# DerrickWang005/CRIS.pytorch

Measured on AMD Instinct MI355X. Metric: train-step samples/sec, CRIS-R50 416x416 bs=64; loss parity vs ref, higher is better.
Workload: dtype bf16; 1 GPU; CRIS-R50 bf16 training step (fwd+BCE+bwd+Adam), 416x416, per-GPU bs=8, 17-token text, synthetic RefCOCO-shape batch resident in HBM (BASELINE.json configs[1]); global_batch=8, parallelism=dp1, launch=graph, graph_captured=True, syncbn_exchange=none, grad_exchange=none

## Files before the change

cris/pytorch_amd/csrc/elementwise.hip:

```cpp
#include <cmath>
#include "common.h"
#include "../../../include/cris_hip.h"

__device__ __forceinline__ void ld8f(const float* p, float* f) {
    const float4 a = *reinterpret_cast<const float4*>(p);
    const float4 b = *reinterpret_cast<const float4*>(p + 4);
    f[0] = a.x; f[1] = a.y; f[2] = a.z; f[3] = a.w; f[4] = b.x; f[5] = b.y; f[6] = b.z; f[7] = b.w;
}
__device__ __forceinline__ void ld8bf(const bf16_t* p, float* f) { unpack8(*reinterpret_cast<const uint4*>(p), f); }
__device__ __forceinline__ void st8bf(bf16_t* p, const float* f) { *reinterpret_cast<uint4*>(p) = pack8(f); }

#define GRID_STRIDE(idx, total) \
    for (long idx = (long)blockIdx.x * blockDim.x + threadIdx.x; idx < (total); idx += (long)gridDim.x * blockDim.x)

__global__ void stem_im2col_kernel(const float* __restrict__ img, int Bn, int H, int W, int OH, int OW, bf16_t* __restrict__ out) {
    const long total = (long)Bn * OH * OW * 4;
    const bool small = total < (1L << 24);
    GRID_STRIDE(idx, total) {
        const cris_idx4 q = cris_split4(idx, 4, OW, OH, small);
        const int kc = q.cv, ow = q.x, oh = q.y, b = q.b;
        const long m = idx >> 2;
        float v[8];
#pragma unroll
        for (int j = 0; j < 8; ++j) {
// ... 41 lines not shown
#pragma unroll
        for (int j = 0; j < 8; ++j) o[j] *= 0.25f;
        st8bf(y + (size_t)mo * ldy + ycoff + cv * 8, o);
    }
}

extern "C" int cris_avgpool2_fwd(const cris_bf16* x, int ldx, int xcoff, int Bn, int H, int W, int C, cris_bf16* y,
                                 int ldy, int ycoff, void* stream) {
    CRIS_CHECK_ARG(x && y && !(H & 1) && !(W & 1) && !(C & 7) && !(ldx & 7) && !(ldy & 7) && !(xcoff & 7) && !(ycoff & 7), "bad args");
    const long total = (long)Bn * (H / 2) * (W / 2) * (C / 8);
    hipLaunchKernelGGL(avgpool2_fwd_kernel, dim3(cris_grid_1d(total, 256)), dim3(256), 0, (hipStream_t)stream, x, ldx, xcoff,
                       Bn, H, W, C, y, ldy, ycoff);
    CRIS_LAUNCH_CHECK();
    return 0;
}

__global__ void avgpool2_bwd_kernel(const bf16_t* __restrict__ dy, int lddy, int dycoff, int Bn, int H, int W, int C,
                                    bf16_t* __restrict__ dx, int lddx, int dxcoff, int accum) {
    const int CV = C >> 3, OH = H >> 1, OW = W >> 1;
    const long total = (long)Bn * H * W * CV;
    const bool small = total < (1L << 24);
    GRID_STRIDE(idx, total) {
        const cris_idx4 q = cris_split4(idx, CV, W, H, small);
        const int cv = q.cv, w = q.x, h = q.y, b = q.b;
        const long m = ((long)b * H + h) * W + w;
        float g[8];
        ld8bf(dy + (((size_t)b * OH + (h >> 1)) * OW + (w >> 1)) * lddy + dycoff + cv * 8, g);
        bf16_t* d = dx + (size_t)m * lddx + dxcoff + cv * 8;
        float o[8];
        if (accum) ld8bf(d, o);
#pragma unroll
        for (int j = 0; j < 8; ++j) o[j] = (accum ? o[j] : 0.f) + 0.25f * g[j];
        st8bf(d, o);
    }
}

extern "C" int cris_avgpool2_bwd(const cris_bf16* dy, int lddy, int dycoff, int Bn, int H, int W, int C, cris_bf16* dx,
                                 int lddx, int dxcoff, int accum, void* stream) {
    CRIS_CHECK_ARG(dy && dx && !(H & 1) && !(W & 1) && !(C & 7) && !(lddx & 7) && !(lddy & 7) && !(dxcoff & 7) && !(dycoff & 7), "bad args");
    const long total = (long)Bn * H * W * (C / 8);
    hipLaunchKernelGGL(avgpool2_bwd_kernel, dim3(cris_grid_1d(total, 256)), dim3(256), 0, (hipStream_t)stream, dy, lddy, dycoff,
                       Bn, H, W, C, dx, lddx, dxcoff, accum);
    CRIS_LAUNCH_CHECK();
    return 0;
}

__device__ __forceinline__ void up2_src(int dst, int n_in, int& i0, int& i1, float& l1) {
    float s = (dst + 0.5f) * 0.5f - 0.5f;
    s = fmaxf(s, 0.f);
    i0 = (int)s;
    i1 = i0 < n_in - 1 ? i0 + 1 : i0;
    l1 = s - (float)i0;
}

__global__ void upsample2_fwd_kernel(const bf16_t* __restrict__ x, int ldx, int xcoff, int Bn, int H, int W, int C,
                                     bf16_t* __restrict__ y, int ldy, int ycoff) {
    const int CV = C >> 3, OH = H * 2, OW = W * 2;
    const long total = (long)Bn * OH * OW * CV;
    const bool small = total < (1L << 24);
    GRID_STRIDE(idx, total) {
        const cris_idx4 q = cris_split4(idx, CV, OW, OH, small);
        const int cv = q.cv, ow = q.x, oh = q.y, b = q.b;
        const long mo = ((long)b * OH + oh) * OW + ow;
        int y0, y1, x0, x1;
        float ly, lx;
        up2_src(oh, H, y0, y1, ly);
        up2_src(ow, W, x0, x1, lx);
        const bf16_t* base = x + (size_t)b * H * W * ldx + xcoff + cv * 8;
        float a[8], bb[8], c[8], d[8], o[8];
        ld8bf(base + ((size_t)y0 * W + x0) * ldx, a);
        ld8bf(base + ((size_t)y0 * W + x1) * ldx, bb);
        ld8bf(base + ((size_t)y1 * W + x0) * ldx, c);
        ld8bf(base + ((size_t)y1 * W + x1) * ldx, d);
        const float w00 = (1.f - ly) * (1.f - lx), w01 = (1.f - ly) * lx, w10 = ly * (1.f - lx), w11 = ly * lx;
#pragma unroll
        for (int j = 0; j < 8; ++j) o[j] = w00 * a[j] + w01 * bb[j] + w10 * c[j] + w11 * d[j];
        st8bf(y + (size_t)mo * ldy + ycoff + cv * 8, o);
    }
}

extern "C" int cris_upsample2_fwd(const cris_bf16* x, int ldx, int xcoff, int Bn, int H, int W, int C, cris_bf16* y,
                                  int ldy, int ycoff, void* stream) {
    CRIS_CHECK_ARG(x && y && !(C & 7) && !(ldx & 7) && !(ldy & 7) && !(xcoff & 7) && !(ycoff & 7), "bad args");
    const long total = (long)Bn * H * W * 4 * (C / 8);
    hipLaunchKernelGGL(upsample2_fwd_kernel, dim3(cris_grid_1d(total, 256)), dim3(256), 0, (hipStream_t)stream, x, ldx, xcoff,
                       Bn, H, W, C, y, ldy, ycoff);
    CRIS_LAUNCH_CHECK();
    return 0;
}

__global__ void upsample2_bwd_kernel(const bf16_t* __restrict__ dy, int lddy, int dycoff, int Bn, int H, int W, int C,
                                     bf16_t* __restrict__ dx, int lddx, int dxcoff, int accum) {
    const int CV = C >> 3, OH = H * 2, OW = W * 2;
    const long total = (long)Bn * H * W * CV;
    const bool small = total < (1L << 24);
    GRID_STRIDE(idx, total) {
        const cris_idx4 q = cris_split4(idx, CV, W, H, small);
        const int cv = q.cv, ix = q.x, iy = q.y, b = q.b;
        const long m = ((long)b * H + iy) * W + ix;
        float acc[8] = {0, 0, 0, 0, 0, 0, 0, 0};
        const bf16_t* base = dy + (size_t)b * OH * OW * lddy + dycoff + cv * 8;
        for (int oy = max(0, 2 * iy - 2); oy <= min(OH - 1, 2 * iy + 2); ++oy) {
            int y0, y1; float ly;
            up2_src(oy, H, y0, y1, ly);
            float wy = 0.f;
            if (y0 == iy) wy += 1.f - ly;
            if (y1 == iy) wy += ly;
            if (wy == 0.f) continue;
            for (int ox = max(0, 2 * ix - 2); ox <= min(OW - 1, 2 * ix + 2); ++ox) {
                int x0, x1; float lx;
                up2_src(ox, W, x0, x1, lx);
                float wx = 0.f;
                if (x0 == ix) wx += 1.f - lx;
                if (x1 == ix) wx += lx;
                if (wx == 0.f) continue;
                float g[8];
                ld8bf(base + ((size_t)oy * OW + ox) * lddy, g);
                const float w = wy * wx;
#pragma unroll
                for (int j = 0; j < 8; ++j) acc[j] += w * g[j];
            }
        }
        bf16_t* d = dx + (size_t)m * lddx + dxcoff + cv * 8;
        if (accum) {
            float o[8];
            ld8bf(d, o);
#pragma unroll
            for (int j = 0; j < 8; ++j) acc[j] += o[j];
        }
        st8bf(d, acc);
    }
}

extern "C" int cris_upsample2_bwd(const cris_bf16* dy, int lddy, int dycoff, int Bn, int H, int W, int C, cris_bf16* dx,
                                  int lddx, int dxcoff, int accum, void* stream) {
    CRIS_CHECK_ARG(dy && dx && !(C & 7) && !(lddx & 7) && !(lddy & 7) && !(dxcoff & 7) && !(dycoff & 7), "bad args");
    const long total = (long)Bn * H * W * (C / 8);
    hipLaunchKernelGGL(upsample2_bwd_kernel, dim3(cris_grid_1d(total, 256)), dim3(256), 0, (hipStream_t)stream, dy, lddy, dycoff,
                       Bn, H, W, C, dx, lddx, dxcoff, accum);
    CRIS_LAUNCH_CHECK();
    return 0;
}

__device__ __forceinline__ float linspace_m1_1(int i, int n) {
    if (n == 1) return -1.f;
    const float step = 2.f / (float)(n - 1);
    return i < n / 2 ? -1.f + step * (float)i : 1.f - step * (float)(n - 1 - i);
}

__global__ void fill_coords_kernel(bf16_t* x, int ldx, int coff, int nfill, int Bn, int H, int W) {
    const long total = (long)Bn * H * W;
    GRID_STRIDE(m, total) {
        const int w = (int)(m % W);
        const int h = (int)((m / W) % H);
        bf16_t* d = x + (size_t)m * ldx + coff;
        d[0] = f2bf(linspace_m1_1(w, W));
        d[1] = f2bf(linspace_m1_1(h, H));
        for (int j = 2; j < nfill; ++j) d[j] = 0;
    }
}

extern "C" int cris_fill_coords(cris_bf16* x, int ldx, int coff, int nfill, int Bn, int H, int W, void* stream) {
    CRIS_CHECK_ARG(x && nfill >= 2, "bad args");
    hipLaunchKernelGGL(fill_coords_kernel, dim3(cris_grid_1d((long)Bn * H * W, 256)), dim3(256), 0, (hipStream_t)stream, x, ldx,
                       coff, nfill, Bn, H, W);
    CRIS_LAUNCH_CHECK();
    return 0;
}

__global__ void gather_samples_kernel(const bf16_t* __restrict__ x, int ldx, int xcoff, const int32_t* __restrict__ index,
                                      int R, int CV, bf16_t* __restrict__ y, int ldy, int ycoff, int total) {
    for (int idx = blockIdx.x * blockDim.x + threadIdx.x; idx < total; idx += gridDim.x * blockDim.x) {
        const int cv = idx % CV;
        const int row = idx / CV;
        const int k = row / R;
// ... 315 lines not shown
    const long total = (long)T * C;
    GRID_STRIDE(idx, total) {
        const int c = (int)(idx % C);
        const int t = (int)(idx / C);
        float s = 0.f;
#pragma unroll 7
        for (int j = 0; j < GG; ++j) s += R[t * GG + j] * pos[(size_t)(1 + j) * C + c];
        posr[idx] = s;
    }
}
extern "C" int cris_posresize_fwd(const float* R, const float* pos, int T, int G, int C, float* posr, void* stream) {
    CRIS_CHECK_ARG(R && pos && posr, "bad args");
    hipLaunchKernelGGL(posresize_fwd_kernel, dim3(cris_grid_1d((long)T * C, 256)), dim3(256), 0, (hipStream_t)stream, R, pos, T,
                       G * G, C, posr);
    CRIS_LAUNCH_CHECK();
    return 0;
}
__global__ void posresize_bwd_kernel(const float* R, const float* dposr, int T, int GG, int C, float* dpos) {
    const long total = (long)GG * C;
    GRID_STRIDE(idx, total) {
        const int c = (int)(idx % C);
        const int j = (int)(idx / C);
        float s = 0.f;
#pragma unroll 13
        for (int t = 0; t < T; ++t) s += R[t * GG + j] * dposr[(size_t)t * C + c];
        dpos[(size_t)(1 + j) * C + c] += s;
    }
}
extern "C" int cris_posresize_bwd(const float* R, const float* dposr, int T, int G, int C, float* dpos, void* stream) {
    CRIS_CHECK_ARG(R && dposr && dpos, "bad args");
    hipLaunchKernelGGL(posresize_bwd_kernel, dim3(cris_grid_1d((long)G * G * C, 256)), dim3(256), 0, (hipStream_t)stream, R,
                       dposr, T, G * G, C, dpos);
    CRIS_LAUNCH_CHECK();
    return 0;
}
__global__ void batch_rowsum_kernel(const bf16_t* dx, int ldx, int Bn, int T, int C, float* out) {
    const long total = (long)T * C;
    GRID_STRIDE(idx, total) {
        const int c = (int)(idx % C);
        const int t = (int)(idx / C);
        float s = 0.f;
        for (int b = 0; b < Bn; ++b) s += bf2f(dx[((size_t)b * T + t) * ldx + c]);
        out[idx] = s;
    }
}
extern "C" int cris_batch_rowsum(const cris_bf16* dx, int ldx, int Bn, int T, int C, float* out, void* stream) {
    CRIS_CHECK_ARG(dx && out, "bad args");
    hipLaunchKernelGGL(batch_rowsum_kernel, dim3(cris_grid_1d((long)T * C, 256)), dim3(256), 0, (hipStream_t)stream, dx, ldx, Bn,
                       T, C, out);
    CRIS_LAUNCH_CHECK();
    return 0;
}

__global__ __launch_bounds__(256) void dynconv_fwd_kernel(const bf16_t* __restrict__ x, int H, int W, int C, const float* __restrict__ wb,
                                                          int ldwb, float* __restrict__ pred, int pix_per_block) {
    const int b = blockIdx.y;
    const int LP = C >> 3;
    const int cl = threadIdx.x % LP, sub = threadIdx.x / LP, nsub = 256 / LP;
    float w[9][8];
    const float* wp = wb + (size_t)b * ldwb;
#pragma unroll
    for (int t = 0; t < 9; ++t)
#pragma unroll
        for (int j = 0; j < 8; ++j) w[t][j] = wp[(cl * 8 + j) * 9 + t];
    const float bias = wp[C * 9];
    const int HW = H * W;
    const int p0 = blockIdx.x * pix_per_block;
    const int p1 = min(HW, p0 + pix_per_block);
    for (int pb = p0; pb < p1; pb += nsub) {
        const int pix = pb + sub;
        float acc = 0.f;
        if (pix < p1) {
            const int oh = pix / W, ow = pix - oh * W;
#pragma unroll
            for (int kh = 0; kh < 3; ++kh)
#pragma unroll
                for (int kw = 0; kw < 3; ++kw) {
                    const int ih = oh + kh - 1, iw = ow + kw - 1;
                    const float ok = ((unsigned)ih < (unsigned)H && (unsigned)iw < (unsigned)W) ? 1.f : 0.f;
                    const int ihc = min(max(ih, 0), H - 1), iwc = min(max(iw, 0), W - 1);
                    float v[8];
                    ld8bf(x + (((size_t)b * H + ihc) * W + iwc) * C + cl * 8, v);
#pragma unroll
                    for (int j = 0; j < 8; ++j) acc += ok * v[j] * w[kh * 3 + kw][j];
                }
        }
        for (int o = LP >> 1; o > 0; o >>= 1) acc += __shfl_xor(acc, o, 64);
        if (cl == 0 && pix < p1) pred[(size_t)b * HW + pix] = acc + bias;
    }
}

extern "C" int cris_dynconv_fwd(const cris_bf16* x, int Bn, int H, int W, int C, const float* wb, int ldwb, float* pred,
                                void* stream) {
    const int LP = C / 8;
    CRIS_CHECK_ARG(x && wb && pred && !(C & 7) && LP >= 1 && LP <= 64 && (LP & (LP - 1)) == 0, "C/8 must be a power of two <= 64");
    constexpr int ppb = 128;
    dim3 grid(cris_cdiv(H * W, ppb), Bn);
    hipLaunchKernelGGL(dynconv_fwd_kernel, grid, dim3(256), 0, (hipStream_t)stream, x, H, W, C, wb, ldwb, pred, ppb);
    CRIS_LAUNCH_CHECK();
    return 0;
}

__global__ __launch_bounds__(256) void dynconv_bwd_kernel(const bf16_t* __restrict__ x, const float* __restrict__ dpred, int H, int W, int C,
                                                          const float* __restrict__ wb, int ldwb, bf16_t* __restrict__ dx,
                                                          float* __restrict__ dwb_part, int pix_per_block) {
    extern __shared__ float sdw[];
    const int b = blockIdx.y;
    const int LP = C >> 3;
    const int cl = threadIdx.x % LP, sub = threadIdx.x / LP, nsub = 256 / LP;
    for (int i = threadIdx.x; i < C * 9 + 1; i += 256) sdw[i] = 0.f;
    __syncthreads();
    float w[9][8], dw[9][8];
    const float* wp = wb + (size_t)b * ldwb;
#pragma unroll
    for (int t = 0; t < 9; ++t)
#pragma unroll
        for (int j = 0; j < 8; ++j) {
            w[t][j] = wp[(cl * 8 + j) * 9 + t];
            dw[t][j] = 0.f;
        }
    float dbias = 0.f;
    const int HW = H * W;
    const float* dp = dpred + (size_t)b * HW;
    const int p0 = blockIdx.x * pix_per_block;
    const int p1 = min(HW, p0 + pix_per_block);
    for (int pix = p0 + sub; pix < p1; pix += nsub) {
        const int ph = pix / W, pw = pix - ph * W;
        float gx[8] = {0, 0, 0, 0, 0, 0, 0, 0};
        const float g0 = dp[pix];
        if (cl == 0) dbias += g0;
        float xq[8];
        ld8bf(x + ((size_t)b * HW + pix) * C + cl * 8, xq);
#pragma unroll
        for (int kh = 0; kh < 3; ++kh)
#pragma unroll
            for (int kw = 0; kw < 3; ++kw) {
                const int oh = ph - kh + 1, ow = pw - kw + 1;
                const float okg = ((unsigned)oh < (unsigned)H && (unsigned)ow < (unsigned)W) ? 1.f : 0.f;
                const float g = okg * dp[min(max(oh, 0), H - 1) * W + min(max(ow, 0), W - 1)];
#pragma unroll
                for (int j = 0; j < 8; ++j) {
                    gx[j] += g * w[kh * 3 + kw][j];
                    dw[kh * 3 + kw][j] += g * xq[j];
                }
            }
        st8bf(dx + ((size_t)b * HW + pix) * C + cl * 8, gx);
    }
    for (int o = LP; o < 64; o <<= 1) {
#pragma unroll
        for (int t = 0; t < 9; ++t)
#pragma unroll
            for (int j = 0; j < 8; ++j) dw[t][j] += __shfl_xor(dw[t][j], o, 64);
        dbias += __shfl_xor(dbias, o, 64);
    }
    const int lane = threadIdx.x & 63;
    for (int w = 0; w < 4; ++w) {
        if ((int)(threadIdx.x >> 6) == w && lane < LP) {
#pragma unroll
            for (int t = 0; t < 9; ++t)
#pragma unroll
                for (int j = 0; j < 8; ++j) sdw[(cl * 8 + j) * 9 + t] += dw[t][j];
            if (cl == 0) sdw[C * 9] += dbias;
        }
        __syncthreads();
    }
    float* part = dwb_part + ((size_t)blockIdx.x * gridDim.y + b) * ldwb;
    for (int i = threadIdx.x; i < ldwb; i += 256) part[i] = i < C * 9 + 1 ? sdw[i] : 0.f;
}

#define DYNCONV_BWD_PPB 128
static int dynconv_bwd_blocks(int HW) { return cris_cdiv(HW, DYNCONV_BWD_PPB); }
extern "C" long cris_dynconv_bwd_ws_floats(int Bn, int H, int W, int ldwb) { return (long)dynconv_bwd_blocks(H * W) * Bn * ldwb; }
void cris_launch_sum_partials(const float* part, int nparts, int ncol, float* out, hipStream_t stream);

extern "C" int cris_dynconv_bwd(const cris_bf16* x, const float* dpred, int Bn, int H, int W, int C, const float* wb, int ldwb,
                                cris_bf16* dx, float* dwb, float* ws, void* stream) {
    const int LP = C / 8;
    CRIS_CHECK_ARG(x && dpred && wb && dx && dwb && ws && !(C & 7) && LP >= 1 && LP <= 64 && (LP & (LP - 1)) == 0 && ldwb >= C * 9 + 1,
                   "bad args");
    const int ppb = DYNCONV_BWD_PPB;
    dim3 grid(dynconv_bwd_blocks(H * W), Bn);
    hipLaunchKernelGGL(dynconv_bwd_kernel, grid, dim3(256), (size_t)(C * 9 + 1) * sizeof(float), (hipStream_t)stream, x, dpred, H, W,
                       C, wb, ldwb, dx, ws, ppb);
    CRIS_LAUNCH_CHECK();
    cris_launch_sum_partials(ws, grid.x, Bn * ldwb, dwb, (hipStream_t)stream);
    CRIS_LAUNCH_CHECK();
    return 0;
}

__global__ void mask_resize_kernel(const float* mask, int Bn, int IH, int IW, int OH, int OW, float* out) {
    const float sh = (float)IH / (float)OH, sw = (float)IW / (float)OW;
    const long total = (long)Bn * OH * OW;
    GRID_STRIDE(idx, total) {
        const int ow = (int)(idx % OW);
        const int oh = (int)((idx / OW) % OH);
        const int b = (int)(idx / ((long)OW * OH));
        const int ih = min((int)floorf(oh * sh), IH - 1);
        const int iw = min((int)floorf(ow * sw), IW - 1);
        out[idx] = mask[((size_t)b * IH + ih) * IW + iw];
    }
}
extern "C" int cris_mask_resize_nearest(const float* mask, int Bn, int IH, int IW, int OH, int OW, float* out, void* stream) {
    CRIS_CHECK_ARG(mask && out, "bad args");
    hipLaunchKernelGGL(mask_resize_kernel, dim3(cris_grid_1d((long)Bn * OH * OW, 256)), dim3(256), 0, (hipStream_t)stream, mask, Bn,
                       IH, IW, OH, OW, out);
    CRIS_LAUNCH_CHECK();
    return 0;
}

#define BCE_BLOCKS 128
__global__ __launch_bounds__(256) void bce_fwd_kernel(const float* x, const float* t, long n, float* part) {
    __shared__ float sw[4];
    float s = 0.f;
    const long n4 = n >> 2;
    for (long i = (long)blockIdx.x * 256 + threadIdx.x; i < n4; i += (long)BCE_BLOCKS * 256) {
        const float4 v = *reinterpret_cast<const float4*>(x + i * 4);
        const float4 y = *reinterpret_cast<const float4*>(t + i * 4);
        s += fmaxf(v.x, 0.f) - v.x * y.x + log1pf(__expf(-fabsf(v.x)));
        s += fmaxf(v.y, 0.f) - v.y * y.y + log1pf(__expf(-fabsf(v.y)));
        s += fmaxf(v.z, 0.f) - v.z * y.z + log1pf(__expf(-fabsf(v.z)));
// ... 537 lines not shown
```

cris/pytorch_amd/csrc/norm.hip:

```cpp
#include "common.h"
#include "../../../include/cris_hip.h"
#include "p2p_ll.h"
#include <string.h>

#define BN_WIDE_MIN 128
#define BN_MERGE_MIN 512
#define BN_MERGE_SLICES 64

template <int PL>
__device__ __forceinline__ float bn_lane_sum(float (*sh)[17], float v, int pl, int cl) {
    __syncthreads();
    sh[pl][cl] = v;
    __syncthreads();
    if (PL == 64) {
        float g = 0.f;
        if (pl < 8) {
#pragma unroll
            for (int j = 0; j < 8; ++j) g += sh[pl * 8 + j][cl];
        }
        __syncthreads();
        if (pl < 8) sh[pl][cl] = g;
        __syncthreads();
    }
    float t = sh[0][cl];
// ... 1049 lines not shown
            p.mean[row] = mean;
            p.rstd[row] = rstd;
        }
#pragma unroll
        for (int i = 0; i < LN_MAXV; ++i) {
            const int c0 = (lane + 64 * i) * 8;
            if (c0 >= p.C) continue;
            float ga[8], be[8], o[8];
            load8f(p.gamma + c0, ga);
            load8f(p.beta + c0, be);
#pragma unroll
            for (int j = 0; j < 8; ++j) o[j] = (v[i][j] - mean) * rstd * ga[j] + be[j];
            const size_t oo = (size_t)row * p.C + c0;
            if (p.y) cris_st16(p.y + oo, pack8(o));
            if (p.ypos) {
                float pe[8], t[8];
                load8f(p.pos + (size_t)(row % p.pos_rows) * p.C + c0, pe);
#pragma unroll
                for (int j = 0; j < 8; ++j) t[j] = o[j] + pe[j];
                cris_st16(p.ypos + oo, pack8(t));
            }
            if (p.out_f32) {
                float r[8];
                if (p.resid) load8f(p.resid + oo, r);
                else {
#pragma unroll
                    for (int j = 0; j < 8; ++j) r[j] = 0.f;
                }
#pragma unroll
                for (int j = 0; j < 8; ++j) {
                    float t = o[j];
                    if (p.out_thresh) t = cris_keep(out_key, (uint32_t)row * (uint32_t)p.C + (uint32_t)(c0 + j), p.out_thresh) ? t * out_scale : 0.f;
                    r[j] += t;
                }
                *reinterpret_cast<float4*>(p.out_f32 + oo) = make_float4(r[0], r[1], r[2], r[3]);
                *reinterpret_cast<float4*>(p.out_f32 + oo + 4) = make_float4(r[4], r[5], r[6], r[7]);
            }
        }
    }
}

extern "C" int cris_ln_fwd(const cris_ln_fwd_params* pp, void* stream) {
    const cris_ln_fwd_params& p = *pp;
    CRIS_CHECK_ARG(p.x && p.gamma && p.beta && p.mean && p.rstd && p.rows > 0, "null operand");
    CRIS_CHECK_ARG((p.C & 7) == 0 && p.C <= 64 * 8 * LN_MAXV && (p.ldx & 7) == 0, "C must be a multiple of 8, <= 2048");
    CRIS_CHECK_ARG(!p.ypos || (p.pos && p.pos_rows > 0), "ypos needs pos");
    CRIS_CHECK_ARG((long)p.rows * p.C < (1L << 32), "dropout index overflow");
    const int grid = cris_grid_1d(p.rows, 4, 2048);
    hipLaunchKernelGGL(ln_fwd_kernel, dim3(grid), dim3(256), 0, (hipStream_t)stream, p);
    CRIS_LAUNCH_CHECK();
    return 0;
}

template <int V>
__global__ __launch_bounds__(256) void ln_bwd_kernel(const cris_ln_bwd_params p) {
    __shared__ float sg[2][64 * 8 * V];
    const int lane = threadIdx.x & 63;
    const int wave_g = blockIdx.x * 4 + (threadIdx.x >> 6);
    const int nwaves = gridDim.x * 4;
    for (int i = threadIdx.x; i < 2 * 64 * 8 * V; i += 256) (&sg[0][0])[i] = 0.f;
    __syncthreads();
    const uint32_t sdev = p.seed_dev ? p.seed_dev[0] : 0u;
    const uint32_t in_key = cris_drop_key(p.in_seed + sdev, p.in_stream);
    const uint32_t out_key = cris_drop_key(p.out_seed + sdev, p.out_stream);
    const float in_scale = p.in_thresh ? 1.f / (1.f - p.in_drop_p) : 1.f;
    const float out_scale = p.out_thresh ? 1.f / (1.f - p.out_drop_p) : 1.f;
    const float invC = 1.f / (float)p.C;
    float dga[V][8], dbe[V][8];
#pragma unroll
    for (int i = 0; i < V; ++i)
#pragma unroll
        for (int j = 0; j < 8; ++j) dga[i][j] = dbe[i][j] = 0.f;

    for (int row = wave_g; row < p.rows; row += nwaves) {
        float v[V][8], msk[V][8];
        ln_load_row<true, V>(p.x, p.x_f32, (size_t)row * p.ldx, p.C, lane, p.in_relu, p.in_thresh, in_scale, in_key, (uint32_t)row,
                          v, msk);
        const float mean = p.mean[row], rstd = p.rstd[row];
        float a[V][8];
        float s1 = 0.f, s2 = 0.f;
#pragma unroll
        for (int i = 0; i < V; ++i) {
            const int c0 = (lane + 64 * i) * 8;
            if (c0 < p.C) {
                const size_t oo = (size_t)row * p.C + c0;
                float g[8], t[8], ga[8];
#pragma unroll
                for (int j = 0; j < 8; ++j) g[j] = 0.f;
                if (p.dy) {
                    load8bf(p.dy + oo, t);
#pragma unroll
                    for (int j = 0; j < 8; ++j) g[j] += t[j];
                }
                if (p.dypos) {
                    load8bf(p.dypos + oo, t);
#pragma unroll
                    for (int j = 0; j < 8; ++j) g[j] += t[j];
                }
                if (p.dout_f32) {
                    load8f(p.dout_f32 + oo, t);
#pragma unroll
                    for (int j = 0; j < 8; ++j) {
                        float d = t[j];
                        if (p.out_thresh) d = cris_keep(out_key, (uint32_t)row * (uint32_t)p.C + (uint32_t)(c0 + j), p.out_thresh) ? d * out_scale : 0.f;
                        g[j] += d;
                    }
                }
                load8f(p.gamma + c0, ga);
#pragma unroll
                for (int j = 0; j < 8; ++j) {
                    const float xh = (v[i][j] - mean) * rstd;
                    v[i][j] = xh;
                    dga[i][j] += g[j] * xh;
                    dbe[i][j] += g[j];
                    a[i][j] = g[j] * ga[j];
                    s1 += a[i][j];
                    s2 += a[i][j] * xh;
                }
            } else {
#pragma unroll
                for (int j = 0; j < 8; ++j) a[i][j] = 0.f;
            }
        }
        const float m1 = wave_sum(s1) * invC, m2 = wave_sum(s2) * invC;
#pragma unroll
        for (int i = 0; i < V; ++i) {
            const int c0 = (lane + 64 * i) * 8;
            if (c0 >= p.C) continue;
            float o[8];
#pragma unroll
            for (int j = 0; j < 8; ++j) o[j] = rstd * (a[i][j] - m1 - v[i][j] * m2) * msk[i][j];
            const size_t xo = (size_t)row * p.ldx + c0;
            if (p.dx_f32) {
                float* d = reinterpret_cast<float*>(p.dx) + xo;
                if (p.dx_accum) {
                    float old[8];
                    load8f(d, old);
#pragma unroll
                    for (int j = 0; j < 8; ++j) o[j] += old[j];
                }
                *reinterpret_cast<float4*>(d) = make_float4(o[0], o[1], o[2], o[3]);
                *reinterpret_cast<float4*>(d + 4) = make_float4(o[4], o[5], o[6], o[7]);
            } else {
                cris_st16(reinterpret_cast<bf16_t*>(p.dx) + xo, pack8(o));
            }
        }
    }
    for (int w = 0; w < 4; ++w) {
        if ((int)(threadIdx.x >> 6) == w) {
#pragma unroll
            for (int i = 0; i < V; ++i) {
                const int c0 = (lane + 64 * i) * 8;
                if (c0 < p.C) {
#pragma unroll
                    for (int j = 0; j < 8; ++j) {
                        sg[0][c0 + j] += dga[i][j];
                        sg[1][c0 + j] += dbe[i][j];
                    }
                }
            }
        }
        __syncthreads();
    }
    float* part = p.part + (size_t)blockIdx.x * 2 * p.C;
    for (int c = threadIdx.x; c < p.C; c += 256) {
        part[c] = sg[0][c];
        part[p.C + c] = sg[1][c];
    }
}

constexpr int LN_BWD_BLOCKS = 512;
static int ln_bwd_grid(int rows) { return cris_grid_1d(rows, 4, LN_BWD_BLOCKS); }
extern "C" int cris_ln_bwd_parts(int rows) { return ln_bwd_grid(rows); }

extern "C" int cris_ln_bwd(const cris_ln_bwd_params* pp, void* stream) {
    const cris_ln_bwd_params& p = *pp;
    CRIS_CHECK_ARG(p.x && p.gamma && p.mean && p.rstd && p.dx && p.part && p.rows > 0, "null operand");
    CRIS_CHECK_ARG(p.dy || p.dypos || p.dout_f32, "no incoming gradient");
    CRIS_CHECK_ARG((p.C & 7) == 0 && p.C <= 64 * 8 * LN_MAXV && (p.ldx & 7) == 0, "C must be a multiple of 8, <= 2048");
    CRIS_CHECK_ARG(!p.dx_accum || p.dx_f32, "accumulate only into fp32");
    static const int narrow = cris_env_int("CRIS_LN_BWD_V", 1);
    const dim3 grid(ln_bwd_grid(p.rows));
    if (narrow && p.C <= 512) hipLaunchKernelGGL(ln_bwd_kernel<1>, grid, dim3(256), 0, (hipStream_t)stream, p);
    else if (narrow && p.C <= 1024) hipLaunchKernelGGL(ln_bwd_kernel<2>, grid, dim3(256), 0, (hipStream_t)stream, p);
    else hipLaunchKernelGGL(ln_bwd_kernel<LN_MAXV>, grid, dim3(256), 0, (hipStream_t)stream, p);
    CRIS_LAUNCH_CHECK();
    return 0;
}

__global__ __launch_bounds__(256) void sum_group_kernel(const cris_sum_group g) {
    __shared__ float sh[4][64];
    int ei = 0;
#pragma unroll
    for (int i = 1; i < CRIS_SUM_GROUP_MAX; ++i) ei += g.block_start[i] <= (int)blockIdx.x ? 1 : 0;
    const cris_sum_entry e = g.e[ei];
    const int cl = threadIdx.x & 63, pl = threadIdx.x >> 6;
    const int c = (blockIdx.x - g.block_start[ei]) * 64 + cl;
    float a = 0.f;
    if (c < e.ncol)
        for (int i = pl; i < e.nparts; i += 4) a += e.part[(size_t)i * e.ld + c];
    sh[pl][cl] = a;
    __syncthreads();
    if (pl == 0 && c < e.ncol) e.out[c] = (sh[0][cl] + sh[1][cl]) + (sh[2][cl] + sh[3][cl]);
}

extern "C" int cris_sum_tables(const cris_sum_group* gp, void* stream) {
    CRIS_CHECK_ARG(gp && gp->n > 0 && gp->n <= CRIS_SUM_GROUP_MAX, "1 .. CRIS_SUM_GROUP_MAX tables per launch");
    cris_sum_group g = *gp;
    int start = 0;
    for (int i = 0; i < g.n; ++i) {
        CRIS_CHECK_ARG(g.e[i].part && g.e[i].out && g.e[i].nparts > 0 && g.e[i].ncol > 0 && g.e[i].ld >= g.e[i].ncol, "bad table");
        g.block_start[i] = start;
        start += cris_cdiv(g.e[i].ncol, 64);
    }
    for (int i = g.n; i <= CRIS_SUM_GROUP_MAX; ++i) g.block_start[i] = start;
    hipLaunchKernelGGL(sum_group_kernel, dim3(start), dim3(256), 0, (hipStream_t)stream, g);
    CRIS_LAUNCH_CHECK();
    return 0;
}
```

Baseline: 679.0 samples/s.

## Restructure upsample, dynconv and layernorm-backward kernels for register reuse and batching

Upsample2 forward now has each thread load one 2x2 source neighbourhood and write the up to four output pixels that share it, instead of doing four loads per output. Upsample2 backward replaces its branchy gather loop with a fixed 4x4 unrolled gather using precomputed weights and predication. Dynconv forward computes runs of 4 adjacent pixels from a shared register window and sizes its grid adaptively. Dynconv backward batches 4 pixels' loads ahead of compute and moves shared-memory dW to a vectorised transposed layout. LayerNorm backward keeps per-wave gamma/beta partials in shared memory instead of registers, packs the dropout mask into bits, and adds a full-width specialisation with occupancy hints. The cost is more register pressure and redundant clamped loads at borders.

Result: no change. 683.5 samples/s (median of 6 runs) (+0.7%).

```diff
diff --git a/cris/pytorch_amd/csrc/elementwise.hip b/cris/pytorch_amd/csrc/elementwise.hip
--- a/cris/pytorch_amd/csrc/elementwise.hip
+++ b/cris/pytorch_amd/csrc/elementwise.hip
@@ -117,37 +117,62 @@
     i1 = i0 < n_in - 1 ? i0 + 1 : i0;
     l1 = s - (float)i0;
 }
+__device__ __forceinline__ float up2_tap(int dst, int n_in, int src) {
+    int i0, i1;
+    float l1;
+    up2_src(dst, n_in, i0, i1, l1);
+    float w = 0.f;
+    if (i0 == src) w += 1.f - l1;
+    if (i1 == src) w += l1;
+    return w;
+}
 
 __global__ void upsample2_fwd_kernel(const bf16_t* __restrict__ x, int ldx, int xcoff, int Bn, int H, int W, int C,
                                      bf16_t* __restrict__ y, int ldy, int ycoff) {
-    const int CV = C >> 3, OH = H * 2, OW = W * 2;
-    const long total = (long)Bn * OH * OW * CV;
+    const int CV = C >> 3, OH = H * 2, OW = W * 2, QH = H + 1, QW = W + 1;
+    const long total = (long)Bn * QH * QW * CV;
     const bool small = total < (1L << 24);
     GRID_STRIDE(idx, total) {
-        const cris_idx4 q = cris_split4(idx, CV, OW, OH, small);
-        const int cv = q.cv, ow = q.x, oh = q.y, b = q.b;
-        const long mo = ((long)b * OH + oh) * OW + ow;
-        int y0, y1, x0, x1;
-        float ly, lx;
-        up2_src(oh, H, y0, y1, ly);
-        up2_src(ow, W, x0, x1, lx);
+        const cris_idx4 q = cris_split4(idx, CV, QW, QH, small);
+        const int cv = q.cv, kx = q.x, ky = q.y, b = q.b;
+        const int r0 = max(ky - 1, 0), r1 = ky == 0 ? min(1, H - 1) : min(ky, H - 1);
+        const int c0 = max(kx - 1, 0), c1 = kx == 0 ? min(1, W - 1) : min(kx, W - 1);
         const bf16_t* base = x + (size_t)b * H * W * ldx + xcoff + cv * 8;
-        float a[8], bb[8], c[8], d[8], o[8];
-        ld8bf(base + ((size_t)y0 * W + x0) * ldx, a);
-        ld8bf(base + ((size_t)y0 * W + x1) * ldx, bb);
-        ld8bf(base + ((size_t)y1 * W + x0) * ldx, c);
-        ld8bf(base + ((size_t)y1 * W + x1) * ldx, d);
-        const float w00 = (1.f - ly) * (1.f - lx), w01 = (1.f - ly) * lx, w10 = ly * (1.f - lx), w11 = ly * lx;
-#pragma unroll
-        for (int j = 0; j < 8; ++j) o[j] = w00 * a[j] + w01 * bb[j] + w10 * c[j] + w11 * d[j];
-        st8bf(y + (size_t)mo * ldy + ycoff + cv * 8, o);
+        float a[8], bb[8], c[8], d[8];
+        ld8bf(base + ((size_t)r0 * W + c0) * ldx, a);
+        ld8bf(base + ((size_t)r0 * W + c1) * ldx, bb);
+        ld8bf(base + ((size_t)r1 * W + c0) * ldx, c);
+        ld8bf(base + ((size_t)r1 * W + c1) * ldx, d);
+#pragma unroll
+        for (int dy = 0; dy < 2; ++dy) {
+            const int oh = 2 * ky - 1 + dy;
+            if (oh < 0 || oh >= OH) continue;
+            int y0, y1;
+            float ly;
+            up2_src(oh, H, y0, y1, ly);
+#pragma unroll
+            for (int dx = 0; dx < 2; ++dx) {
+                const int ow = 2 * kx - 1 + dx;
+                if (ow < 0 || ow >= OW) continue;
+                int x0, x1;
+                float lx;
+                up2_src(ow, W, x0, x1, lx);
+                const float w00 = (1.f - ly) * (1.f - lx), w01 = (1.f - ly) * lx, w10 = ly * (1.f - lx), w11 = ly * lx;
+                float o[8];
+#pragma unroll
+                for (int j = 0; j < 8; ++j) o[j] = w00 * a[j] + w01 * bb[j] + w10 * c[j] + w11 * d[j];
+                const long mo = ((long)b * OH + oh) * OW + ow;
+                st8bf(y + (size_t)mo * ldy + ycoff + cv * 8, o);
+            }
+        }
     }
 }
 
 extern "C" int cris_upsample2_fwd(const cris_bf16* x, int ldx, int xcoff, int Bn, int H, int W, int C, cris_bf16* y,
                                   int ldy, int ycoff, void* stream) {
     CRIS_CHECK_ARG(x && y && !(C & 7) && !(ldx & 7) && !(ldy & 7) && !(xcoff & 7) && !(ycoff & 7), "bad args");
-    const long total = (long)Bn * H * W * 4 * (C / 8);
+    if (Bn <= 0 || H <= 0 || W <= 0 || C <= 0) return 0;
+    const long total = (long)Bn * (H + 1) * (W + 1) * (C / 8);
     hipLaunchKernelGGL(upsample2_fwd_kernel, dim3(cris_grid_1d(total, 256)), dim3(256), 0, (hipStream_t)stream, x, ldx, xcoff,
                        Bn, H, W, C, y, ldy, ycoff);
     CRIS_LAUNCH_CHECK();
@@ -165,27 +190,38 @@
         const long m = ((long)b * H + iy) * W + ix;
         float acc[8] = {0, 0, 0, 0, 0, 0, 0, 0};
         const bf16_t* base = dy + (size_t)b * OH * OW * lddy + dycoff + cv * 8;
-        for (int oy = max(0, 2 * iy - 2); oy <= min(OH - 1, 2 * iy + 2); ++oy) {
-            int y0, y1; float ly;
-            up2_src(oy, H, y0, y1, ly);
-            float wy = 0.f;
-            if (y0 == iy) wy += 1.f - ly;
-            if (y1 == iy) wy += ly;
-            if (wy == 0.f) continue;
-            for (int ox = max(0, 2 * ix - 2); ox <= min(OW - 1, 2 * ix + 2); ++ox) {
-                int x0, x1; float lx;
-                up2_src(ox, W, x0, x1, lx);
-                float wx = 0.f;
-                if (x0 == ix) wx += 1.f - lx;
-                if (x1 == ix) wx += lx;
-                if (wx == 0.f) continue;
+        int oyc[4], oxc[4];
+        float wy[4], wx[4];
+        bool oky[4], okx[4];
+#pragma unroll
+        for (int t = 0; t < 4; ++t) {
+            const int oy = 2 * iy - 1 + t, ox = 2 * ix - 1 + t;
+            oky[t] = oy >= 0 && oy < OH;
+            okx[t] = ox >= 0 && ox < OW;
+            oyc[t] = min(max(oy, 0), OH - 1);
+            oxc[t] = min(max(ox, 0), OW - 1);
+            wy[t] = up2_tap(oyc[t], H, iy);
+            wx[t] = up2_tap(oxc[t], W, ix);
+        }
+        uint4 gv[4][4];
+#pragma unroll
+        for (int ty = 0; ty < 4; ++ty)
+#pragma unroll
+            for (int tx = 0; tx < 4; ++tx) gv[ty][tx] = *reinterpret_cast<const uint4*>(base + ((size_t)oyc[ty] * OW + oxc[tx]) * lddy);
+#pragma unroll
+        for (int ty = 0; ty < 4; ++ty)
+#pragma unroll
+            for (int tx = 0; tx < 4; ++tx) {
                 float g[8];
-                ld8bf(base + ((size_t)oy * OW + ox) * lddy, g);
-                const float w = wy * wx;
-#pragma unroll
-                for (int j = 0; j < 8; ++j) acc[j] += w * g[j];
+                unpack8(gv[ty][tx], g);
+                const float w = wy[ty] * wx[tx];
+                const bool ok = oky[ty] && okx[tx];
+#pragma unroll
+                for (int j = 0; j < 8; ++j) {
+                    const float s = acc[j] + w * g[j];
+                    acc[j] = ok ? s : acc[j];
+                }
             }
-        }
         bf16_t* d = dx + (size_t)m * lddx + dxcoff + cv * 8;
         if (accum) {
             float o[8];
@@ -607,8 +643,10 @@
     return 0;
 }
 
+#define DYNCONV_RUN 4
 __global__ __launch_bounds__(256) void dynconv_fwd_kernel(const bf16_t* __restrict__ x, int H, int W, int C, const float* __restrict__ wb,
-                                                          int ldwb, float* __restrict__ pred, int pix_per_block) {
+                                                          int ldwb, float* __restrict__ pred, int runs_per_block) {
+    constexpr int T = DYNCONV_RUN;
     const int b = blockIdx.y;
     const int LP = C >> 3;
     const int cl = threadIdx.x % LP, sub = threadIdx.x / LP, nsub = 256 / LP;
@@ -620,28 +658,44 @@
         for (int j = 0; j < 8; ++j) w[t][j] = wp[(cl * 8 + j) * 9 + t];
     const float bias = wp[C * 9];
     const int HW = H * W;
-    const int p0 = blockIdx.x * pix_per_block;
-    const int p1 = min(HW, p0 + pix_per_block);
-    for (int pb = p0; pb < p1; pb += nsub) {
-        const int pix = pb + sub;
-        float acc = 0.f;
-        if (pix < p1) {
-            const int oh = pix / W, ow = pix - oh * W;
+    const int WR = (W + T - 1) / T;
+    const int r0 = blockIdx.x * runs_per_block;
+    const int r1 = min(H * WR, r0 + runs_per_block);
+    for (int rb = r0; rb < r1; rb += nsub) {
+        const int run = rb + sub;
+        const bool act = run < r1;
+        const int oh = act ? run / WR : 0, ow0 = act ? (run - oh * WR) * T : 0;
+        float acc[T];
+#pragma unroll
+        for (int t = 0; t < T; ++t) acc[t] = 0.f;
+        if (act) {
+            uint4 xv[3][T + 2];
 #pragma unroll
             for (int kh = 0; kh < 3; ++kh)
 #pragma unroll
-                for (int kw = 0; kw < 3; ++kw) {
-                    const int ih = oh + kh - 1, iw = ow + kw - 1;
-                    const float ok = ((unsigned)ih < (unsigned)H && (unsigned)iw < (unsigned)W) ? 1.f : 0.f;
-                    const int ihc = min(max(ih, 0), H - 1), iwc = min(max(iw, 0), W - 1);
-                    float v[8];
-                    ld8bf(x + (((size_t)b * H + ihc) * W + iwc) * C + cl * 8, v);
-#pragma unroll
-                    for (int j = 0; j < 8; ++j) acc += ok * v[j] * w[kh * 3 + kw][j];
+                for (int c = 0; c < T + 2; ++c) {
+                    const int ihc = min(max(oh + kh - 1, 0), H - 1), iwc = min(max(ow0 + c - 1, 0), W - 1);
+                    xv[kh][c] = *reinterpret_cast<const uint4*>(x + (((size_t)b * H + ihc) * W + iwc) * C + cl * 8);
                 }
-        }
-        for (int o = LP >> 1; o > 0; o >>= 1) acc += __shfl_xor(acc, o, 64);
-        if (cl == 0 && pix < p1) pred[(size_t)b * HW + pix] = acc + bias;
+#pragma unroll
+            for (int t = 0; t < T; ++t)
+#pragma unroll
+                for (int kh = 0; kh < 3; ++kh)
+#pragma unroll
+                    for (int kw = 0; kw < 3; ++kw) {
+                        const int ih = oh + kh - 1, iw = ow0 + t + kw - 1;
+                        const float ok = ((unsigned)ih < (unsigned)H && (unsigned)iw < (unsigned)W) ? 1.f : 0.f;
+                        float v[8];
+                        unpack8(xv[kh][t + kw], v);
+#pragma unroll
+                        for (int j = 0; j < 8; ++j) acc[t] += ok * v[j] * w[kh * 3 + kw][j];
+                    }
+        }
+#pragma unroll
+        for (int t = 0; t < T; ++t) {
+            for (int o = LP >> 1; o > 0; o >>= 1) acc[t] += __shfl_xor(acc[t], o, 64);
+            if (cl == 0 && act && ow0 + t < W) pred[(size_t)b * HW + oh * W + ow0 + t] = acc[t] + bias;
+        }
     }
 }
 
@@ -649,17 +703,22 @@
                                 void* stream) {
     const int LP = C / 8;
     CRIS_CHECK_ARG(x && wb && pred && !(C & 7) && LP >= 1 && LP <= 64 && (LP & (LP - 1)) == 0, "C/8 must be a power of two <= 64");
-    constexpr int ppb = 128;
-    dim3 grid(cris_cdiv(H * W, ppb), Bn);
-    hipLaunchKernelGGL(dynconv_fwd_kernel, grid, dim3(256), 0, (hipStream_t)stream, x, H, W, C, wb, ldwb, pred, ppb);
-    CRIS_LAUNCH_CHECK();
-    return 0;
-}
-
+    CRIS_CHECK_ARG(Bn > 0 && H > 0 && W > 0, "empty operand");
+    const int nsub = 256 / LP, runs = H * cris_cdiv(W, DYNCONV_RUN);
+    int rpb = cris_cdiv((long)runs * Bn, 512);
+    if (rpb < 32) rpb = 32;
+    rpb = cris_cdiv(rpb, nsub) * nsub;
+    dim3 grid(cris_cdiv(runs, rpb), Bn);
+    hipLaunchKernelGGL(dynconv_fwd_kernel, grid, dim3(256), 0, (hipStream_t)stream, x, H, W, C, wb, ldwb, pred, rpb);
+    CRIS_LAUNCH_CHECK();
+    return 0;
+}
+
+#define DYNCONV_BWD_BATCH 4
 __global__ __launch_bounds__(256) void dynconv_bwd_kernel(const bf16_t* __restrict__ x, const float* __restrict__ dpred, int H, int W, int C,
                                                           const float* __restrict__ wb, int ldwb, bf16_t* __restrict__ dx,
                                                           float* __restrict__ dwb_part, int pix_per_block) {
-    extern __shared__ float sdw[];
+    extern __shared__ __attribute__((aligned(16))) float sdw[];
     const int b = blockIdx.y;
     const int LP = C >> 3;
     const int cl = threadIdx.x % LP, sub = threadIdx.x / LP, nsub = 256 / LP;
@@ -679,27 +738,40 @@
     const float* dp = dpred + (size_t)b * HW;
     const int p0 = blockIdx.x * pix_per_block;
     const int p1 = min(HW, p0 + pix_per_block);
-    for (int pix = p0 + sub; pix < p1; pix += nsub) {
-        const int ph = pix / W, pw = pix - ph * W;
-        float gx[8] = {0, 0, 0, 0, 0, 0, 0, 0};
-        const float g0 = dp[pix];
-        if (cl == 0) dbias += g0;
-        float xq[8];
-        ld8bf(x + ((size_t)b * HW + pix) * C + cl * 8, xq);
-#pragma unroll
-        for (int kh = 0; kh < 3; ++kh)
-#pragma unroll
-            for (int kw = 0; kw < 3; ++kw) {
-                const int oh = ph - kh + 1, ow = pw - kw + 1;
-                const float okg = ((unsigned)oh < (unsigned)H && (unsigned)ow < (unsigned)W) ? 1.f : 0.f;
-                const float g = okg * dp[min(max(oh, 0), H - 1) * W + min(max(ow, 0), W - 1)];
+    constexpr int D = DYNCONV_BWD_BATCH;
+    for (int pb = p0 + sub; pb < p1; pb += nsub * D) {
+        uint4 xr[D];
+        float g[D][9];
+#pragma unroll
+        for (int d = 0; d < D; ++d) {
+            const int pix = min(pb + d * nsub, p1 - 1);
+            const int ph = pix / W, pw = pix - ph * W;
+            xr[d] = *reinterpret_cast<const uint4*>(x + ((size_t)b * HW + pix) * C + cl * 8);
+#pragma unroll
+            for (int kh = 0; kh < 3; ++kh)
+#pragma unroll
+                for (int kw = 0; kw < 3; ++kw) {
+                    const int oh = ph - kh + 1, ow = pw - kw + 1;
+                    const float okg = ((unsigned)oh < (unsigned)H && (unsigned)ow < (unsigned)W) ? 1.f : 0.f;
+                    g[d][kh * 3 + kw] = okg * dp[min(max(oh, 0), H - 1) * W + min(max(ow, 0), W - 1)];
+                }
+        }
+#pragma unroll
+        for (int d = 0; d < D; ++d) {
+            const int pix = pb + d * nsub;
+            if (pix >= p1) break;
+            float gx[8] = {0, 0, 0, 0, 0, 0, 0, 0}, xq[8];
+            unpack8(xr[d], xq);
+            if (cl == 0) dbias += g[d][4];
+#pragma unroll
+            for (int t = 0; t < 9; ++t)
 #pragma unroll
                 for (int j = 0; j < 8; ++j) {
-                    gx[j] += g * w[kh * 3 + kw][j];
-                    dw[kh * 3 + kw][j] += g * xq[j];
+                    gx[j] += g[d][t] * w[t][j];
+                    dw[t][j] += g[d][t] * xq[j];
                 }
-            }
-        st8bf(dx + ((size_t)b * HW + pix) * C + cl * 8, gx);
+            st8bf(dx + ((size_t)b * HW + pix) * C + cl * 8, gx);
+        }
     }
     for (int o = LP; o < 64; o <<= 1) {
 #pragma unroll
@@ -712,15 +784,23 @@
     for (int w = 0; w < 4; ++w) {
         if ((int)(threadIdx.x >> 6) == w && lane < LP) {
 #pragma unroll
-            for (int t = 0; t < 9; ++t)
-#pragma unroll
-                for (int j = 0; j < 8; ++j) sdw[(cl * 8 + j) * 9 + t] += dw[t][j];
+            for (int t = 0; t < 9; ++t) {
+                float4* q = reinterpret_cast<float4*>(sdw + t * C + cl * 8);
+                float4 lo = q[0], hi = q[1];
+                lo.x += dw[t][0]; lo.y += dw[t][1]; lo.z += dw[t][2]; lo.w += dw[t][3];
+                hi.x += dw[t][4]; hi.y += dw[t][5]; hi.z += dw[t][6]; hi.w += dw[t][7];
+                q[0] = lo;
+                q[1] = hi;
+            }
             if (cl == 0) sdw[C * 9] += dbias;
         }
         __syncthreads();
     }
     float* part = dwb_part + ((size_t)blockIdx.x * gridDim.y + b) * ldwb;
-    for (int i = threadIdx.x; i < ldwb; i += 256) part[i] = i < C * 9 + 1 ? sdw[i] : 0.f;
+    for (int i = threadIdx.x; i < ldwb; i += 256) {
+        const int c = i / 9;
+        part[i] = i < C * 9 ? sdw[(i - c * 9) * C + c] : i == C * 9 ? sdw[i] : 0.f;
+    }
 }
 
 #define DYNCONV_BWD_PPB 128
diff --git a/cris/pytorch_amd/csrc/norm.hip b/cris/pytorch_amd/csrc/norm.hip
--- a/cris/pytorch_amd/csrc/norm.hip
+++ b/cris/pytorch_amd/csrc/norm.hip
@@ -1125,75 +1125,152 @@
     return 0;
 }
 
-template <int V>
-__global__ __launch_bounds__(256) void ln_bwd_kernel(const cris_ln_bwd_params p) {
-    __shared__ float sg[2][64 * 8 * V];
+__device__ __forceinline__ void load8f4(const float* lo, const float* hi, float* f) {
+    const float4 a = *reinterpret_cast<const float4*>(lo), b = *reinterpret_cast<const float4*>(hi);
+    f[0] = a.x; f[1] = a.y; f[2] = a.z; f[3] = a.w; f[4] = b.x; f[5] = b.y; f[6] = b.z; f[7] = b.w;
+}
+
+template <int V, bool FULL>
+__global__ __launch_bounds__(256, !FULL ? 1 : V == 4 ? 2 : V == 2 ? 3 : 4) void ln_bwd_kernel(const cris_ln_bwd_params p) {
+    __shared__ float sg[4][2][64 * 8 * V];
     const int lane = threadIdx.x & 63;
     const int wave_g = blockIdx.x * 4 + (threadIdx.x >> 6);
     const int nwaves = gridDim.x * 4;
-    for (int i = threadIdx.x; i < 2 * 64 * 8 * V; i += 256) (&sg[0][0])[i] = 0.f;
-    __syncthreads();
+    float* accg = sg[threadIdx.x >> 6][0] + lane * 4;
+    float* accb = sg[threadIdx.x >> 6][1] + lane * 4;
+#pragma unroll
+    for (int s = 0; s < 2 * V; ++s) {
+        *reinterpret_cast<float4*>(accg + s * 256) = make_float4(0.f, 0.f, 0.f, 0.f);
+        *reinterpret_cast<float4*>(accb + s * 256) = make_float4(0.f, 0.f, 0.f, 0.f);
+    }
     const uint32_t sdev = p.seed_dev ? p.seed_dev[0] : 0u;
     const uint32_t in_key = cris_drop_key(p.in_seed + sdev, p.in_stream);
     const uint32_t out_key = cris_drop_key(p.out_seed + sdev, p.out_stream);
     const float in_scale = p.in_thresh ? 1.f / (1.f - p.in_drop_p) : 1.f;
     const float out_scale = p.out_thresh ? 1.f / (1.f - p.out_drop_p) : 1.f;
+    const float mscale = p.in_thresh ? 1.f * in_scale : 1.f;
     const float invC = 1.f / (float)p.C;
-    float dga[V][8], dbe[V][8];
-#pragma unroll
-    for (int i = 0; i < V; ++i)
-#pragma unroll
-        for (int j = 0; j < 8; ++j) dga[i][j] = dbe[i][j] = 0.f;
+    int cc[V];
+    bool live[V];
+#pragma unroll
+    for (int i = 0; i < V; ++i) {
+        const int c0 = (lane + 64 * i) * 8;
+        live[i] = FULL || c0 < p.C;
+        cc[i] = live[i] ? c0 : 0;
+    }
 
     for (int row = wave_g; row < p.rows; row += nwaves) {
-        float v[V][8], msk[V][8];
-        ln_load_row<true, V>(p.x, p.x_f32, (size_t)row * p.ldx, p.C, lane, p.in_relu, p.in_thresh, in_scale, in_key, (uint32_t)row,
-                          v, msk);
+        const size_t xrow = (size_t)row * p.ldx, orow = (size_t)row * p.C;
+        uint4 rx[V][2], rg[V];
+        if (p.x_f32) {
+#pragma unroll
+            for (int i = 0; i < V; ++i) {
+                const uint4* s = reinterpret_cast<const uint4*>(reinterpret_cast<const float*>(p.x) + xrow + cc[i]);
+                rx[i][0] = s[0];
+                rx[i][1] = s[1];
+            }
+        } else {
+#pragma unroll
+            for (int i = 0; i < V; ++i) rx[i][0] = *reinterpret_cast<const uint4*>(reinterpret_cast<const bf16_t*>(p.x) + xrow + cc[i]);
+        }
+        if (p.dy) {
+#pragma unroll
+            for (int i = 0; i < V; ++i) rg[i] = *reinterpret_cast<const uint4*>(p.dy + orow + cc[i]);
+        }
         const float mean = p.mean[row], rstd = p.rstd[row];
+
+        float v[V][8];
+        uint32_t mbits = 0u;
+#pragma unroll
+        for (int i = 0; i < V; ++i) {
+            if (p.x_f32) {
+                v[i][0] = __uint_as_float(rx[i][0].x); v[i][1] = __uint_as_float(rx[i][0].y);
+                v[i][2] = __uint_as_float(rx[i][0].z); v[i][3] = __uint_as_float(rx[i][0].w);
+                v[i][4] = __uint_as_float(rx[i][1].x); v[i][5] = __uint_as_float(rx[i][1].y);
+                v[i][6] = __uint_as_float(rx[i][1].z); v[i][7] = __uint_as_float(rx[i][1].w);
+            } else {
+                unpack8(rx[i][0], v[i]);
+            }
+#pragma unroll
+            for (int j = 0; j < 8; ++j) {
+                float m = 1.f;
+                if (p.in_relu && !(v[i][j] > 0.f)) m = 0.f;
+                if (p.in_thresh) m = cris_keep(in_key, (uint32_t)row * (uint32_t)p.C + (uint32_t)(cc[i] + j), p.in_thresh) ? m * in_scale : 0.f;
+                float vm = v[i][j] * m;
+                asm volatile("" : "+v"(vm));
+                v[i][j] = live[i] ? vm : 0.f;
+                mbits |= (live[i] && m != 0.f) ? 1u << (i * 8 + j) : 0u;
+            }
+        }
+        float g[V][8];
+#pragma unroll
+        for (int i = 0; i < V; ++i)
+#pragma unroll
+            for (int j = 0; j < 8; ++j) g[i][j] = 0.f;
+        if (p.dy) {
+#pragma unroll
+            for (int i = 0; i < V; ++i) {
+                float t[8];
+                unpack8(rg[i], t);
+#pragma unroll
+                for (int j = 0; j < 8; ++j) g[i][j] += t[j];
+            }
+        }
+        if (p.dypos) {
+            uint4 r[V];
+#pragma unroll
+            for (int i = 0; i < V; ++i) r[i] = *reinterpret_cast<const uint4*>(p.dypos + orow + cc[i]);
+#pragma unroll
+            for (int i = 0; i < V; ++i) {
+                float t[8];
+                unpack8(r[i], t);
+#pragma unroll
+                for (int j = 0; j < 8; ++j) g[i][j] += t[j];
+            }
+        }
+        if (p.dout_f32) {
+            float4 r[V][2];
+#pragma unroll
+            for (int i = 0; i < V; ++i) {
+                r[i][0] = *reinterpret_cast<const float4*>(p.dout_f32 + orow + cc[i]);
+                r[i][1] = *reinterpret_cast<const float4*>(p.dout_f32 + orow + cc[i] + 4);
+            }
+#pragma unroll
+            for (int i = 0; i < V; ++i) {
+                const float t[8] = {r[i][0].x, r[i][0].y, r[i][0].z, r[i][0].w, r[i][1].x, r[i][1].y, r[i][1].z, r[i][1].w};
+#pragma unroll
+                for (int j = 0; j < 8; ++j) {
+                    float d = t[j];
+                    if (p.out_thresh) d = cris_keep(out_key, (uint32_t)row * (uint32_t)p.C + (uint32_t)(cc[i] + j), p.out_thresh) ? d * out_scale : 0.f;
+                    g[i][j] += d;
+                }
+            }
+        }
         float a[V][8];
         float s1 = 0.f, s2 = 0.f;
 #pragma unroll
         for (int i = 0; i < V; ++i) {
-            const int c0 = (lane + 64 * i) * 8;
-            if (c0 < p.C) {
-                const size_t oo = (size_t)row * p.C + c0;
-                float g[8], t[8], ga[8];
-#pragma unroll
-                for (int j = 0; j < 8; ++j) g[j] = 0.f;
-                if (p.dy) {
-                    load8bf(p.dy + oo, t);
-#pragma unroll
-                    for (int j = 0; j < 8; ++j) g[j] += t[j];
-                }
-                if (p.dypos) {
-                    load8bf(p.dypos + oo, t);
-#pragma unroll
-                    for (int j = 0; j < 8; ++j) g[j] += t[j];
-                }
-                if (p.dout_f32) {
-                    load8f(p.dout_f32 + oo, t);
-#pragma unroll
-                    for (int j = 0; j < 8; ++j) {
-                        float d = t[j];
-                        if (p.out_thresh) d = cris_keep(out_key, (uint32_t)row * (uint32_t)p.C + (uint32_t)(c0 + j), p.out_thresh) ? d * out_scale : 0.f;
-                        g[j] += d;
-                    }
-                }
-                load8f(p.gamma + c0, ga);
-#pragma unroll
-                for (int j = 0; j < 8; ++j) {
-                    const float xh = (v[i][j] - mean) * rstd;
-                    v[i][j] = xh;
-                    dga[i][j] += g[j] * xh;
-                    dbe[i][j] += g[j];
-                    a[i][j] = g[j] * ga[j];
-                    s1 += a[i][j];
-                    s2 += a[i][j] * xh;
-                }
-            } else {
-#pragma unroll
-                for (int j = 0; j < 8; ++j) a[i][j] = 0.f;
-            }
+            float ga[8], dga[8], dbe[8];
+            load8f(p.gamma + cc[i], ga);
+            load8f4(accg + i * 512, accg + i * 512 + 256, dga);
+            load8f4(accb + i * 512, accb + i * 512 + 256, dbe);
+#pragma unroll
+            for (int j = 0; j < 8; ++j) {
+                const float xh = (v[i][j] - mean) * rstd;
+                const float aj = g[i][j] * ga[j];
+                const float nga = dga[j] + g[i][j] * xh, nbe = dbe[j] + g[i][j];
+                const float n1 = s1 + aj, n2 = s2 + aj * xh;
+                v[i][j] = xh;
+                dga[j] = live[i] ? nga : dga[j];
+                dbe[j] = live[i] ? nbe : dbe[j];
+                a[i][j] = live[i] ? aj : 0.f;
+                s1 = live[i] ? n1 : s1;
+                s2 = live[i] ? n2 : s2;
+            }
+            *reinterpret_cast<float4*>(accg + i * 512) = make_float4(dga[0], dga[1], dga[2], dga[3]);
+            *reinterpret_cast<float4*>(accg + i * 512 + 256) = make_float4(dga[4], dga[5], dga[6], dga[7]);
+            *reinterpret_cast<float4*>(accb + i * 512) = make_float4(dbe[0], dbe[1], dbe[2], dbe[3]);
+            *reinterpret_cast<float4*>(accb + i * 512 + 256) = make_float4(dbe[4], dbe[5], dbe[6], dbe[7]);
         }
         const float m1 = wave_sum(s1) * invC, m2 = wave_sum(s2) * invC;
 #pragma unroll
@@ -1202,7 +1279,7 @@
             if (c0 >= p.C) continue;
             float o[8];
 #pragma unroll
-            for (int j = 0; j < 8; ++j) o[j] = rstd * (a[i][j] - m1 - v[i][j] * m2) * msk[i][j];
+            for (int j = 0; j < 8; ++j) o[j] = rstd * (a[i][j] - m1 - v[i][j] * m2) * ((mbits >> (i * 8 + j)) & 1u ? mscale : 0.f);
             const size_t xo = (size_t)row * p.ldx + c0;
             if (p.dx_f32) {
                 float* d = reinterpret_cast<float*>(p.dx) + xo;
@@ -1219,32 +1296,30 @@
             }
         }
     }
-    for (int w = 0; w < 4; ++w) {
-        if ((int)(threadIdx.x >> 6) == w) {
-#pragma unroll
-            for (int i = 0; i < V; ++i) {
-                const int c0 = (lane + 64 * i) * 8;
-                if (c0 < p.C) {
-#pragma unroll
-                    for (int j = 0; j < 8; ++j) {
-                        sg[0][c0 + j] += dga[i][j];
-                        sg[1][c0 + j] += dbe[i][j];
-                    }
-                }
-            }
-        }
-        __syncthreads();
-    }
+    __syncthreads();
     float* part = p.part + (size_t)blockIdx.x * 2 * p.C;
     for (int c = threadIdx.x; c < p.C; c += 256) {
-        part[c] = sg[0][c];
-        part[p.C + c] = sg[1][c];
+        const int slot = (((c >> 9) * 2 + ((c >> 2) & 1)) * 64 + ((c >> 3) & 63)) * 4 + (c & 3);
+        float sa = 0.f, sb = 0.f;
+#pragma unroll
+        for (int w = 0; w < 4; ++w) {
+            sa += sg[w][0][slot];
+            sb += sg[w][1][slot];
+        }
+        part[c] = sa;
+        part[p.C + c] = sb;
     }
 }
 
 constexpr int LN_BWD_BLOCKS = 512;
 static int ln_bwd_grid(int rows) { return cris_grid_1d(rows, 4, LN_BWD_BLOCKS); }
 extern "C" int cris_ln_bwd_parts(int rows) { return ln_bwd_grid(rows); }
+
+template <int V>
+static void ln_bwd_launch(const cris_ln_bwd_params& p, dim3 grid, hipStream_t stream) {
+    if (p.C == 512 * V) hipLaunchKernelGGL((ln_bwd_kernel<V, true>), grid, dim3(256), 0, stream, p);
+    else hipLaunchKernelGGL((ln_bwd_kernel<V, false>), grid, dim3(256), 0, stream, p);
+}
 
 extern "C" int cris_ln_bwd(const cris_ln_bwd_params* pp, void* stream) {
     const cris_ln_bwd_params& p = *pp;
@@ -1254,9 +1329,9 @@
     CRIS_CHECK_ARG(!p.dx_accum || p.dx_f32, "accumulate only into fp32");
     static const int narrow = cris_env_int("CRIS_LN_BWD_V", 1);
     const dim3 grid(ln_bwd_grid(p.rows));
-    if (narrow && p.C <= 512) hipLaunchKernelGGL(ln_bwd_kernel<1>, grid, dim3(256), 0, (hipStream_t)stream, p);
-    else if (narrow && p.C <= 1024) hipLaunchKernelGGL(ln_bwd_kernel<2>, grid, dim3(256), 0, (hipStream_t)stream, p);
-    else hipLaunchKernelGGL(ln_bwd_kernel<LN_MAXV>, grid, dim3(256), 0, (hipStream_t)stream, p);
+    if (narrow && p.C <= 512) ln_bwd_launch<1>(p, grid, (hipStream_t)stream);
+    else if (narrow && p.C <= 1024) ln_bwd_launch<2>(p, grid, (hipStream_t)stream);
+    else ln_bwd_launch<LN_MAXV>(p, grid, (hipStream_t)stream);
     CRIS_LAUNCH_CHECK();
     return 0;
 }
```
